# rgcgithub/regenie

Hardware: NVIDIA H100
Metric: step1_level0_snps_per_sec (higher is better)
Workload: dtype int8 Gram + int8 prediction (both exact integer sums) + tf32x3 factorisation + f64 refinement / statistics

## Files before the change

regenie_b200/csrc/chol_mixed.cu:

```cuda
#include <algorithm>

#include "gemm_dmma.cuh"
#include "kernels.cuh"

namespace rg {

namespace {

constexpr int PT = 128;
constexpr int PLD = 132;
constexpr int PB = 32;
constexpr int kMxRowsPerCta = 64;

__device__ __forceinline__ void blk_nt(float (&acc)[PB], const float* __restrict__ Arow, const float* __restrict__ Bt, int plen) {
  for (int p0 = 0; p0 < plen; p0 += 4) {
    const float4 a = *reinterpret_cast<const float4*>(Arow + p0);
#pragma unroll
    for (int n = 0; n < PB; ++n) {
      const float4 b = *reinterpret_cast<const float4*>(Bt + n * PLD + p0);
      acc[n] = fmaf(a.x, b.x, acc[n]);
      acc[n] = fmaf(a.y, b.y, acc[n]);
      acc[n] = fmaf(a.z, b.z, acc[n]);
      acc[n] = fmaf(a.w, b.w, acc[n]);
    }
  }
}

}

__global__ void __launch_bounds__(256)
potrf128_kernel(float* __restrict__ Lplain, float* __restrict__ Mplain, float* __restrict__ MTplain, int n, int k,
                unsigned int* __restrict__ fail_flag) {
  extern __shared__ float pt_sm[];
  float* S = pt_sm;
  float* Wm = pt_sm + PT * PLD;
  float* Wq = pt_sm + 2 * PT * PLD;
  float* dinv = pt_sm + 3 * PT * PLD;
  float* lcol = dinv + PT;
  const int warp = threadIdx.x >> 5, lane = threadIdx.x & 31;
  float* Lkk = Lplain + (int64_t)blockIdx.x * n * n + (int64_t)k * PT * n + (int64_t)k * PT;
#pragma unroll
  for (int it = 0; it < PT * PT / 4 / 256; ++it) {
    const int e = threadIdx.x + 256 * it;
    const int r = e >> 5, c = (e & 31) * 4;
    float4 v = *reinterpret_cast<const float4*>(Lkk + (int64_t)r * n + c);
    if (c + 0 > r) v.x = 0.f;
    if (c + 1 > r) v.y = 0.f;
    if (c + 2 > r) v.z = 0.f;
    if (c + 3 > r) v.w = 0.f;
    *reinterpret_cast<float4*>(S + r * PLD + c) = v;
    *reinterpret_cast<float4*>(Wm + r * PLD + c) = make_float4(0.f, 0.f, 0.f, 0.f);
    *reinterpret_cast<float4*>(Wq + r * PLD + c) = make_float4(0.f, 0.f, 0.f, 0.f);
  }
  __syncthreads();
  bool bad = false;
  for (int jb = 0; jb < PT / PB; ++jb) {
    const int j0 = jb * PB;
    if (warp == 0) {
      float a[PB];
#pragma unroll
      for (int c = 0; c < PB; ++c) a[c] = (c <= lane) ? S[(j0 + lane) * PLD + j0 + c] : 0.f;
      float d = __shfl_sync(0xffffffffu, a[0], 0);
#pragma unroll
      for (int c = 0; c < PB; ++c) {
        if (!(d > 0.f)) bad = true;
        float inv = rsqrtf(d);
        inv = inv * (1.5f - 0.5f * d * inv * inv);
        const float l = a[c] * inv;
        a[c] = l;
        if (lane == c) dinv[j0 + c] = inv;
        if (c + 1 < PB) {
          float* lb = lcol + (c & 1) * PB;
          lb[lane] = l;
          d = __shfl_sync(0xffffffffu, fmaf(-l, l, a[c + 1]), c + 1);
          __syncwarp();
          float lv[PB];
#pragma unroll
          for (int q = (c + 1) / 4; q < PB / 4; ++q) {
            const float4 t4 = *reinterpret_cast<const float4*>(lb + 4 * q);
            lv[4 * q] = t4.x; lv[4 * q + 1] = t4.y; lv[4 * q + 2] = t4.z; lv[4 * q + 3] = t4.w;
          }
#pragma unroll
          for (int cc = c + 1; cc < PB; ++cc) a[cc] = fmaf(-l, lv[cc], a[cc]);
        }
      }
#pragma unroll
      for (int c = 0; c < PB; ++c) S[(j0 + lane) * PLD + j0 + c] = a[c];
    }
    __syncthreads();
    if (warp >= 1 && warp < PT / PB - jb) {
      const int i0 = (jb + warp) * PB;
      float x[PB];
#pragma unroll
      for (int c = 0; c < PB; ++c) x[c] = S[(i0 + lane) * PLD + j0 + c];
#pragma unroll
      for (int c = 0; c < PB; ++c) {
        const float* lrow = S + (j0 + c) * PLD + j0;
        float s = x[c];
#pragma unroll
        for (int p = 0; p < c; ++p) s = fmaf(-x[p], lrow[p], s);
        x[c] = s * dinv[j0 + c];
      }
#pragma unroll
      for (int c = 0; c < PB; ++c) S[(i0 + lane) * PLD + j0 + c] = x[c];
    }
    __syncthreads();
    {
      const int nb = PT / PB - jb - 1;
      int t = 0;
      for (int a1 = 0; a1 < nb; ++a1)
        for (int a2 = 0; a2 <= a1; ++a2, ++t) {
          if ((t & 7) != warp) continue;
          const int ib = jb + 1 + a1, i2 = jb + 1 + a2;
          float acc[PB];
#pragma unroll
          for (int c = 0; c < PB; ++c) acc[c] = 0.f;
          blk_nt(acc, S + (ib * PB + lane) * PLD + j0, S + (i2 * PB) * PLD + j0, PB);
          float* o = S + (ib * PB + lane) * PLD + i2 * PB;
#pragma unroll
          for (int c = 0; c < PB; ++c) o[c] -= acc[c];
        }
    }
    __syncthreads();
  }
  if (bad && lane == 0) atomicOr(fail_flag, 2u);
  if (warp < PT / PB) {
    const int j0 = warp * PB;
    float x[PB];
#pragma unroll
    for (int r = 0; r < PB; ++r) {
      const float* lrow = S + (j0 + r) * PLD + j0;
      float s = (r == lane) ? 1.f : 0.f;
#pragma unroll
      for (int p = 0; p < r; ++p) s = fmaf(-lrow[p], x[p], s);
      x[r] = s * dinv[j0 + r];
    }
#pragma unroll
    for (int r = 0; r < PB; ++r) {
      Wm[(j0 + r) * PLD + j0 + lane] = x[r];
      Wq[(j0 + lane) * PLD + j0 + r] = x[r];
    }
  }
  __syncthreads();
  for (int sb = 1; sb < PT / PB; sb *= 2) {
    const int npair = PT / PB / (2 * sb);
    for (int t = warp; t < npair * sb * sb; t += 8) {
      const int pr = t / (sb * sb), bi = (t / sb) % sb, aj = t % sb;
      const int a0 = pr * 2 * sb, b0 = a0 + sb;
      float acc[PB];
#pragma unroll
      for (int c = 0; c < PB; ++c) acc[c] = 0.f;
      blk_nt(acc, S + ((b0 + bi) * PB + lane) * PLD + (a0 + aj) * PB, Wq + ((a0 + aj) * PB) * PLD + (a0 + aj) * PB, (sb - aj) * PB);
#pragma unroll
      for (int c = 0; c < PB; ++c) S[((a0 + aj) * PB + c) * PLD + (b0 + bi) * PB + lane] = acc[c];
    }
    __syncthreads();
    for (int t = warp; t < npair * sb * sb; t += 8) {
      const int pr = t / (sb * sb), bi = (t / sb) % sb, aj = t % sb;
      const int a0 = pr * 2 * sb, b0 = a0 + sb;
      float acc[PB];
#pragma unroll
      for (int c = 0; c < PB; ++c) acc[c] = 0.f;
      blk_nt(acc, Wm + ((b0 + bi) * PB + lane) * PLD + b0 * PB, S + ((a0 + aj) * PB) * PLD + b0 * PB, (bi + 1) * PB);
#pragma unroll
      for (int c = 0; c < PB; ++c) {
        Wm[((b0 + bi) * PB + lane) * PLD + (a0 + aj) * PB + c] = -acc[c];
        Wq[((a0 + aj) * PB + c) * PLD + (b0 + bi) * PB + lane] = -acc[c];
      }
    }
    __syncthreads();
  }
  float* Mp = Mplain + ((int64_t)blockIdx.x * (n / PT) + k) * PT * PT;
  float* MTp = MTplain + ((int64_t)blockIdx.x * (n / PT) + k) * PT * PT;
#pragma unroll 4
  for (int it = 0; it < PT * PT / 4 / 256; ++it) {
    const int e = threadIdx.x + 256 * it;
    const int r = e >> 5, c = (e & 31) * 4;
    float4 vl = *reinterpret_cast<const float4*>(S + r * PLD + c);
    if (c + 0 > r) vl.x = 0.f;
    if (c + 1 > r) vl.y = 0.f;
    if (c + 2 > r) vl.z = 0.f;
    if (c + 3 > r) vl.w = 0.f;
    *reinterpret_cast<float4*>(Lkk + (int64_t)r * n + c) = vl;
    *reinterpret_cast<float4*>(Mp + r * PT + c) = *reinterpret_cast<const float4*>(Wm + r * PLD + c);
    *reinterpret_cast<float4*>(MTp + r * PT + c) = *reinterpret_cast<const float4*>(Wq + r * PLD + c);
  }
}

constexpr float kMxSafety = 64.f;
__device__ __forceinline__ bool mx_finished(const unsigned int* conv, int nmat, int m, int upto_step, float tol) {
  const bool strict = tol < 0.f;
  const float t = fabsf(tol);
  for (int s = 1; s <= upto_step; ++s) {
    const float dx = __uint_as_float(conv[((int64_t)s * nmat + m) * 2]);
    const float xx = __uint_as_float(conv[((int64_t)s * nmat + m) * 2 + 1]);
    if (dx <= t * xx) return true;
    if (!strict && kMxSafety * dx * dx <= t * xx * xx) return true;
  }
  return false;
}

template <int PMAX>
__global__ void __launch_bounds__(256, 2)
mx_residual_kernel(const double* __restrict__ Af, const double* __restrict__ lambda, int R, const double* __restrict__ bvec,
                   const double* __restrict__ xvec, double* __restrict__ rvec, int n, int P, int Pp, int nmat, int step,
                   const unsigned int* __restrict__ conv, float tol) {
  extern __shared__ double rs_sm[];
  const int m = blockIdx.y;
  if (step > 1 && mx_finished(conv, nmat, m, step - 1, tol)) return;
  const int f = m / R;
  const double lam = lambda[m % R];
  const double* x = xvec + (int64_t)m * Pp * n;
  for (int e = threadIdx.x * 2; e < P * n; e += 512) *reinterpret_cast<double2*>(rs_sm + e) = *reinterpret_cast<const double2*>(x + e);
  __syncthreads();
  const int warp = threadIdx.x >> 5, lane = threadIdx.x & 31;
  for (int rg = 0; rg < kMxRowsPerCta / 32; ++rg) {
  const int i0 = blockIdx.x * kMxRowsPerCta + rg * 32 + warp * 4;
  const double* a0 = Af + ((int64_t)f * n + i0) * n;
  double acc[4][PMAX];
#pragma unroll
  for (int a = 0; a < 4; ++a)
#pragma unroll
    for (int p = 0; p < PMAX; ++p) acc[a][p] = 0.0;
  double2 an2[4];
#pragma unroll
  for (int a = 0; a < 4; ++a) an2[a] = *reinterpret_cast<const double2*>(a0 + (int64_t)a * n + lane * 2);
  for (int j = lane * 2; j < n; j += 64) {
    double2 av[4];
#pragma unroll
    for (int a = 0; a < 4; ++a) av[a] = an2[a];
    if (j + 64 < n) {
#pragma unroll
      for (int a = 0; a < 4; ++a) an2[a] = *reinterpret_cast<const double2*>(a0 + (int64_t)a * n + j + 64);
    }
#pragma unroll
    for (int p = 0; p < PMAX; ++p) {
      if (p < P) {
        const double2 b = *reinterpret_cast<const double2*>(rs_sm + p * n + j);
#pragma unroll
        for (int a = 0; a < 4; ++a) acc[a][p] = fma(av[a].x, b.x, fma(av[a].y, b.y, acc[a][p]));
      }
    }
  }
#pragma unroll
  for (int a = 0; a < 4; ++a)
#pragma unroll
    for (int p = 0; p < PMAX; ++p) {
#pragma unroll
      for (int o = 16; o > 0; o >>= 1) acc[a][p] += __shfl_xor_sync(0xffffffffu, acc[a][p], o);
    }
  if (lane == 0) {
#pragma unroll
    for (int a = 0; a < 4; ++a)
#pragma unroll
      for (int p = 0; p < PMAX; ++p)
        if (p < P)
          rvec[((int64_t)m * Pp + p) * n + i0 + a] = bvec[((int64_t)f * Pp + p) * n + i0 + a] - lam * rs_sm[p * n + i0 + a] - acc[a][p];
  }
  }
}


constexpr int RF_ROWS = 64;
constexpr int RF_NV = 64;

__global__ void __launch_bounds__(256)
mx_residual_fused_kernel(const double* __restrict__ Af, const double* __restrict__ lambda, int R, const double* __restrict__ bvec,
                         const double* __restrict__ xvec, double* __restrict__ rvec, int n, int P, int Pp, int nmat, int step,
                         const unsigned int* __restrict__ conv, float tol) {
  __shared__ double As[64 * DM_LD], Bs[64 * DM_LD];
  const int f = blockIdx.y;
  if (step > 1) {
    bool all_done = true;
    for (int r = 0; r < R; ++r) all_done = all_done && mx_finished(conv, nmat, f * R + r, step - 1, tol);
    if (all_done) return;
  }
  const int NV = R * P;
  const int row0 = blockIdx.x * RF_ROWS;
  const int lrow = threadIdx.x >> 2, lp = (threadIdx.x & 3) * 4;
  const bool vb = lrow < NV;
  const double* ap = Af + ((int64_t)f * n + row0 + lrow) * n + lp;
  const double* bp = xvec + ((int64_t)(f * R + (vb ? lrow / P : 0)) * Pp + (vb ? lrow % P : 0)) * n + lp;
  DmmaAcc acc;
  gemm_tile_nt_dmma_ptr(ap, true, bp, vb, n, acc, As, Bs);
#pragma unroll
  for (int j = 0; j < 4; ++j)
#pragma unroll
    for (int e = 0; e < 2; ++e) {
      const int vec = dm_col(j) + e;
      if (vec < NV) {
        const int r = vec / P, p = vec % P, m = f * R + r;
        const double lam = lambda[r];
#pragma unroll
        for (int i = 0; i < 2; ++i) {
          const int row = row0 + dm_row(i);
          const int64_t o = ((int64_t)m * Pp + p) * n + row;
          rvec[o] = bvec[((int64_t)f * Pp + p) * n + row] - lam * xvec[o] - acc.c[i][j][e];
        }
      }
    }
}

constexpr int TS_STAGES = 6;
constexpr int TS_SUB = 32;
constexpr int TS_STAGE_BYTES = TS_SUB * PT * 4;
constexpr int TS_VP = 12;
constexpr int TS_CW = 16;

__device__ __forceinline__ uint32_t ts_smem_u32(const void* p) { return (uint32_t)__cvta_generic_to_shared(p); }
__device__ __forceinline__ void ts_mbar_wait(uint32_t bar, uint32_t parity) {
  uint32_t done = 0, spins = 0;
  while (true) {
    asm volatile(
        "{\n\t.reg .pred p;\n\t"
        "mbarrier.try_wait.parity.shared::cta.b64 p, [%1], %2;\n\t"
        "selp.u32 %0, 1, 0, p;\n\t}"
        : "=r"(done) : "r"(bar), "r"(parity) : "memory");
    if (done) break;
    if (++spins > (1u << 28)) __trap();
  }
}

template <int PMAX>
__global__ void __launch_bounds__(32 * (TS_CW + 1))
mx_trisolve_kernel(const __grid_constant__ CUtensorMap tmL, const __grid_constant__ CUtensorMap tmM,
                   const __grid_constant__ CUtensorMap tmMT, const double* __restrict__ rvec, int64_t r_mat_stride,
                   int r_mat_div, double* __restrict__ xvec, int n, int P, int Pp, int nmat, int step,
                   unsigned int* __restrict__ conv, float tol) {
  constexpr int TS_PARTS = TS_CW / 4;
  constexpr int TS_CPP = TS_SUB / TS_PARTS;
  constexpr int TS_THREADS = 32 * (TS_CW + 1);
  extern __shared__ uint8_t ts_raw[];
  const int m = blockIdx.x;
  if (step > 1 && mx_finished(conv, nmat, m, step - 1, tol)) return;
  const uint32_t raw = ts_smem_u32(ts_raw);
  const uint32_t base = (raw + 127u) & ~127u;
  uint8_t* gen = ts_raw + (base - raw);
  float* tiles = reinterpret_cast<float*>(gen);
  float* v = reinterpret_cast<float*>(gen + TS_STAGES * TS_STAGE_BYTES);
  float* sbuf = v + (size_t)n * TS_VP;
  float* comb = sbuf + PT * TS_VP;
  uint64_t* bars = reinterpret_cast<uint64_t*>(comb + (TS_PARTS - 1) * PT * TS_VP);
  const uint32_t full_bar = ts_smem_u32(bars), empty_bar = ts_smem_u32(bars + TS_STAGES);
  const int warp = threadIdx.x >> 5, lane = threadIdx.x & 31;
  const int nt = n / PT;
  if (threadIdx.x == 0) {
    for (int s = 0; s < TS_STAGES; ++s) {
      asm volatile("mbarrier.init.shared::cta.b64 [%0], %1;" ::"r"(full_bar + 8 * s), "r"(1) : "memory");
      asm volatile("mbarrier.init.shared::cta.b64 [%0], %1;" ::"r"(empty_bar + 8 * s), "r"(TS_CW) : "memory");
    }
    asm volatile("fence.mbarrier_init.release.cluster;" ::: "memory");
    asm volatile("fence.proxy.async.shared::cta;" ::: "memory");
  }
  const double* r = rvec + (int64_t)(r_mat_div > 0 ? m / r_mat_div : m) * r_mat_stride;
  for (int e = threadIdx.x; e < n * TS_VP; e += TS_THREADS) {
    const int i = e / TS_VP, p = e % TS_VP;
    v[e] = p < P ? (float)r[(int64_t)p * n + i] : 0.f;
  }
  __syncthreads();

  if (warp == TS_CW) {
    if (lane == 0) {
      asm volatile("prefetch.tensormap [%0];" ::"l"(&tmL) : "memory");
      asm volatile("prefetch.tensormap [%0];" ::"l"(&tmM) : "memory");
      asm volatile("prefetch.tensormap [%0];" ::"l"(&tmMT) : "memory");
      int it = 0;
      auto push = [&](const CUtensorMap* tm, int c0, int c1) {
        const int s = it % TS_STAGES;
        const uint32_t ph = (it / TS_STAGES) & 1;
        ts_mbar_wait(empty_bar + 8 * s, ph ^ 1);
        asm volatile("mbarrier.arrive.expect_tx.shared::cta.b64 _, [%0], %1;" ::"r"(full_bar + 8 * s), "r"(TS_STAGE_BYTES) : "memory");
        asm volatile(
            "cp.async.bulk.tensor.2d.shared::cluster.global.mbarrier::complete_tx::bytes [%0], [%1, {%3, %4}], [%2];"
            ::"r"(base + s * TS_STAGE_BYTES), "l"(tm), "r"(full_bar + 8 * s), "r"(c0), "r"(c1) : "memory");
        ++it;
      };
      for (int sweep = 0; sweep < 2; ++sweep)
        for (int kk = 0; kk < nt; ++kk) {
          const int k = sweep == 0 ? kk : nt - 1 - kk;
          const int j0 = sweep == 0 ? 0 : k + 1, j1 = sweep == 0 ? k : nt;
          for (int j = j0; j < j1; ++j)
            for (int sub = 0; sub < PT / TS_SUB; ++sub) push(&tmL, k * PT, m * n + j * PT + sub * TS_SUB);
          for (int sub = 0; sub < PT / TS_SUB; ++sub)
            push(sweep == 0 ? &tmMT : &tmM, 0, (m * nt + k) * PT + sub * TS_SUB);
        }
    }
    return;
  }

  const int half = warp >> 2;
  const int row = (warp & 3) * 32 + lane;
  int it = 0;
  float acc[PMAX];
  auto consume = [&](const float* vec ) {
    const int s = it % TS_STAGES;
    const uint32_t ph = (it / TS_STAGES) & 1;
    ts_mbar_wait(full_bar + 8 * s, ph);
    const float* t = tiles + (size_t)s * (TS_STAGE_BYTES / 4) + (size_t)(half * TS_CPP) * PT + row;
    const float* y = vec + (size_t)(half * TS_CPP) * TS_VP;
#pragma unroll
    for (int c = 0; c < TS_CPP; ++c) {
      const float tv = t[(size_t)c * PT];
      const float4 y0 = *reinterpret_cast<const float4*>(y + c * TS_VP);
      const float4 y1 = *reinterpret_cast<const float4*>(y + c * TS_VP + 4);
      const float4 y2 = *reinterpret_cast<const float4*>(y + c * TS_VP + 8);
      const float yy[12] = {y0.x, y0.y, y0.z, y0.w, y1.x, y1.y, y1.z, y1.w, y2.x, y2.y, y2.z, y2.w};
#pragma unroll
      for (int p = 0; p < PMAX; ++p) acc[p] = fmaf(tv, yy[p], acc[p]);
    }
    __syncwarp();
    if (lane == 0) asm volatile("mbarrier.arrive.shared::cta.b64 _, [%0];" ::"r"(empty_bar + 8 * s) : "memory");
    ++it;
  };
  auto consumer_sync = [&]() { asm volatile("bar.sync 1, %0;" ::"n"(32 * TS_CW) : "memory"); };

  for (int sweep = 0; sweep < 2; ++sweep)
    for (int kk = 0; kk < nt; ++kk) {
      const int k = sweep == 0 ? kk : nt - 1 - kk;
      const int j0 = sweep == 0 ? 0 : k + 1, j1 = sweep == 0 ? k : nt;
#pragma unroll
      for (int p = 0; p < PMAX; ++p) acc[p] = 0.f;
      for (int j = j0; j < j1; ++j)
        for (int sub = 0; sub < PT / TS_SUB; ++sub) consume(v + (size_t)(j * PT + sub * TS_SUB) * TS_VP);
      if (half > 0) {
#pragma unroll
        for (int p = 0; p < PMAX; ++p) comb[((half - 1) * PT + row) * TS_VP + p] = acc[p];
      }
      consumer_sync();
      if (half == 0) {
#pragma unroll
        for (int p = 0; p < PMAX; ++p) {
          float sum = acc[p];
#pragma unroll
          for (int h = 0; h < TS_PARTS - 1; ++h) sum += comb[(h * PT + row) * TS_VP + p];
          sbuf[row * TS_VP + p] = v[(size_t)(k * PT + row) * TS_VP + p] - sum;
        }
      }
      consumer_sync();
#pragma unroll
      for (int p = 0; p < PMAX; ++p) acc[p] = 0.f;
      for (int sub = 0; sub < PT / TS_SUB; ++sub) consume(sbuf + (size_t)(sub * TS_SUB) * TS_VP);
      if (half > 0) {
#pragma unroll
        for (int p = 0; p < PMAX; ++p) comb[((half - 1) * PT + row) * TS_VP + p] = acc[p];
      }
      consumer_sync();
      if (half == 0) {
#pragma unroll
        for (int p = 0; p < PMAX; ++p) {
          float sum = acc[p];
#pragma unroll
          for (int h = 0; h < TS_PARTS - 1; ++h) sum += comb[(h * PT + row) * TS_VP + p];
          v[(size_t)(k * PT + row) * TS_VP + p] = sum;
        }
      }
      consumer_sync();
    }

  float dmax = 0.f, xmax = 0.f;
  for (int e = threadIdx.x; e < P * n; e += 32 * TS_CW) {
    const int p = e / n, i = e % n;
    double* xp = xvec + ((int64_t)m * Pp + p) * n + i;
    const float dx = v[(size_t)i * TS_VP + p];
    const double xn = (step == 0 ? 0.0 : *xp) + (double)dx;
    *xp = xn;
    dmax = (fabsf(dx) <= 3.0e38f) ? fmaxf(dmax, fabsf(dx)) : __int_as_float(0x7f800000);
    xmax = fmaxf(xmax, fabsf((float)xn));
  }
  if (step > 0) {
#pragma unroll
    for (int o = 16; o > 0; o >>= 1) {
      dmax = fmaxf(dmax, __shfl_xor_sync(0xffffffffu, dmax, o));
      xmax = fmaxf(xmax, __shfl_xor_sync(0xffffffffu, xmax, o));
    }
    if (lane == 0) {
      atomicMax(conv + ((int64_t)step * nmat + m) * 2, __float_as_uint(dmax));
      atomicMax(conv + ((int64_t)step * nmat + m) * 2 + 1, __float_as_uint(xmax));
    }
  }
}

__global__ void mx_final_check_kernel(const unsigned int* __restrict__ conv, int nmat, int steps, float tol,
                                      unsigned int* __restrict__ fail_flag) {
  const int m = blockIdx.x * blockDim.x + threadIdx.x;
  if (m >= nmat) return;
  bool ok = mx_finished(conv, nmat, m, steps, tol);
  for (int s = 1; s <= steps; ++s) {
    const float dx = __uint_as_float(conv[((int64_t)s * nmat + m) * 2]);
    if (!(dx == dx) || !(fabsf(dx) <= 3.0e38f)) ok = false;
  }
  if (!ok) atomicOr(fail_flag, 1u);
}

struct MxPlan {
  int n = 0, nt = 0;
  DevBuf<int4> tiles;
  std::vector<int2> upd, trsm;
};

static void build_plan(MxPlan& pl, int n) {
  pl.n = n;
  const int nt = n / PT;
  pl.nt = nt;
  std::vector<int4> all;
  pl.upd.clear(); pl.trsm.clear();
  for (int k = 0; k < nt; ++k) {
    int2 u{(int)all.size(), 0};
    for (int i = k; i < nt; ++i) all.push_back(make_int4(i, k, 0, 4 * k));
    u.y = (int)all.size() - u.x;
    pl.upd.push_back(u);
    int2 t{(int)all.size(), 0};
    for (int i = k + 1; i < nt; ++i) all.push_back(make_int4(i, k, 4 * k, 4));
    t.y = (int)all.size() - t.x;
    pl.trsm.push_back(t);
  }
  pl.tiles.alloc(all.size());
  RG_CUDA(cudaMemcpy(pl.tiles.p, all.data(), all.size() * sizeof(int4), cudaMemcpyHostToDevice));
}

struct MixedSolver::Impl {
  int n = 0, nmat = 0, K = 0, R = 0, Pp = 0;
  DevBuf<float> Lplain, Mplain, MTplain, Ap;
  DevBuf<unsigned int> conv;
  CUtensorMap tmL, tmM, tmAp;
  CUtensorMap tmLpl, tmMpl, tmMTpl;
  MxPlan plan;
};

MixedSolver::MixedSolver() : impl(new Impl()) {}
MixedSolver::~MixedSolver() { delete impl; }

int MixedSolver::dim_for(int bs) {
  int n = PT;
  while (n < bs) n *= 2;
  return n <= 2048 ? n : 0;
}

void MixedSolver::prepare(int n, int K, int R, int Pp) {
  Impl& d = *impl;
  const int nmat = K * R;
  if (d.n == n && d.nmat == nmat && d.Pp == Pp) return;
  RG_CHECK(n % PT == 0 && n >= PT && ((n / PT) & (n / PT - 1)) == 0 && n <= 2048,
           "mixed solver: dimension must be 128 * 2^k <= 2048");
  d.n = n; d.nmat = nmat; d.K = K; d.R = R; d.Pp = Pp;
  d.Lplain.alloc((size_t)nmat * n * n);
  d.Mplain.alloc((size_t)nmat * n * PT);
  d.MTplain.alloc((size_t)nmat * n * PT);
  make_f32_rows_tensor_map(&d.tmLpl, d.Lplain.p, n, (int64_t)nmat * n, PT, TS_SUB);
  make_f32_rows_tensor_map(&d.tmMpl, d.Mplain.p, PT, (int64_t)nmat * n, PT, TS_SUB);
  make_f32_rows_tensor_map(&d.tmMTpl, d.MTplain.p, PT, (int64_t)nmat * n, PT, TS_SUB);
  RG_CUDA(cudaMemset(d.Lplain.p, 0, (size_t)nmat * n * n * 4));
  d.conv.alloc((size_t)(kMxMaxSteps + 1) * nmat * 2);
  make_tf32_operand_tensor_map(&d.tmL, d.Lplain.p, n, n, nmat);
  make_tf32_operand_tensor_map(&d.tmM, d.Mplain.p, PT, n, nmat);
  d.Ap.alloc((size_t)K * n * n);
  RG_CUDA(cudaMemset(d.Ap.p, 0, (size_t)K * n * n * 4));
  make_tf32_operand_tensor_map(&d.tmAp, d.Ap.p, n, n, K);
  build_plan(d.plan, n);
}

static int rhs_chunk(int n) { return std::max(1, std::min(12, (int)(98304 / (8 * (size_t)n)))); }

int MixedSolver::launches_per_solve(int n, int steps, int P) {
  const int nt = n / PT;
  const int nch = (P + rhs_chunk(n) - 1) / rhs_chunk(n);
  return 3 * nt - 1 + nch * (1 + 2 * steps) + 1;
}

void MixedSolver::solve(const double* Af, const double* lambda, const double* bvec, double* xvec, double* rvec, int P,
                        int steps, float tol, unsigned int* fail_flag, cudaStream_t s, bool first_col_ready) {
  Impl& d = *impl;
  const int n = d.n, nmat = d.nmat, nt = d.plan.nt;
  RG_CHECK(n > 0, "mixed solver: prepare() first");
  RG_CHECK(P <= d.Pp, "mixed solver: more right-hand sides than the row pitch");
  RG_CHECK(steps >= 1 && steps <= kMxMaxSteps, "mixed solver: bad step count");
  const size_t potrf_smem = ((size_t)3 * PT * PLD + PT + 2 * PB) * sizeof(float);
  ensure_dyn_smem(reinterpret_cast<const void*>(potrf128_kernel), potrf_smem);
  ensure_dyn_smem(reinterpret_cast<const void*>(mx_residual_kernel<12>), 98304);
  ensure_dyn_smem(reinterpret_cast<const void*>(mx_residual_kernel<10>), 98304);
  RG_CHECK(n <= 2048, "mixed solver: n <= 2048");
  const size_t sm_t = (size_t)TS_STAGES * TS_STAGE_BYTES + ((size_t)n + (1 + TS_CW / 4) * PT) * TS_VP * sizeof(float) + 2 * TS_STAGES * 8 + 256;
  ensure_dyn_smem(reinterpret_cast<const void*>(mx_trisolve_kernel<12>), sm_t);
  ensure_dyn_smem(reinterpret_cast<const void*>(mx_trisolve_kernel<10>), sm_t);
  RG_CUDA(cudaMemsetAsync(d.conv.p, 0, d.conv.n * sizeof(unsigned int), s));
  const int4* tl = d.plan.tiles.p;
  Tf32GemmEpilogue e0{};
  e0.n = n; e0.out_mat_stride = (int64_t)n * n; e0.out = d.Lplain.p;
  for (int k = 0; k < nt; ++k) {
    Tf32GemmEpilogue e = e0;
    e.c_chunks = 4; e.c_mat_div = d.R;
    e.diag_add = lambda; e.diag_mod = d.R;
    if (!(k == 0 && first_col_ready)) launch_tf32x3_gemm(d.tmL, d.tmL, tl + d.plan.upd[k].x, d.plan.upd[k].y, nmat, e, s, &d.tmAp);
    potrf128_kernel<<<nmat, 256, potrf_smem, s>>>(d.Lplain.p, d.Mplain.p, d.MTplain.p, n, k, fail_flag);
    if (d.plan.trsm[k].y > 0) {
      Tf32GemmEpilogue t = e0;
      t.mirror = 1;
      t.b_cols_local = 1;
      launch_tf32x3_gemm(d.tmL, d.tmM, tl + d.plan.trsm[k].x, d.plan.trsm[k].y, nmat, t, s);
    }
  }
  dim3 grid(n / kMxRowsPerCta, nmat);
  const int pc = rhs_chunk(n);
  for (int st = 0; st <= steps; ++st)
    for (int p0 = 0; p0 < P; p0 += pc) {
      const int np = std::min(pc, P - p0);
      const size_t sm_r = (size_t)np * n * sizeof(double);
      const int64_t o = (int64_t)p0 * n;
      auto tri = [&](const double* rv, int64_t rs, int rdiv, int step) {
#define RG_TRI(PM) mx_trisolve_kernel<PM><<<nmat, 32 * (TS_CW + 1), sm_t, s>>>(d.tmLpl, d.tmMpl, d.tmMTpl, rv, rs, rdiv, xvec + o, n, np, d.Pp, nmat, step, d.conv.p, tol)
        if (np <= 10) RG_TRI(10);
        else RG_TRI(12);
#undef RG_TRI
      };
      if (st == 0) {
        tri(bvec + o, (int64_t)d.Pp * n, d.R, 0);
      } else {
        if (d.R * np <= RF_NV && n % RF_ROWS == 0)
          mx_residual_fused_kernel<<<dim3(n / RF_ROWS, d.K), 256, 0, s>>>(Af, lambda, d.R, bvec + o, xvec + o, rvec + o, n, np, d.Pp, nmat, st, d.conv.p, tol);
        else if (np <= 10) mx_residual_kernel<10><<<grid, 256, sm_r, s>>>(Af, lambda, d.R, bvec + o, xvec + o, rvec + o, n, np, d.Pp, nmat, st, d.conv.p, tol);
        else mx_residual_kernel<12><<<grid, 256, sm_r, s>>>(Af, lambda, d.R, bvec + o, xvec + o, rvec + o, n, np, d.Pp, nmat, st, d.conv.p, tol);
        tri(rvec + o, (int64_t)d.Pp * n, 0, st);
      }
    }
  mx_final_check_kernel<<<(nmat + 63) / 64, 64, 0, s>>>(d.conv.p, nmat, steps, tol, fail_flag);
}

float* MixedSolver::a_planes() { return impl->Ap.p; }
float* MixedSolver::l_planes() { return impl->Lplain.p; }

const float* MixedSolver::debug_planes(int which) const {
  switch (which) {
    case 2: return impl->Lplain.p;
    case 3: return impl->Mplain.p;
    default: return nullptr;
  }
}

}
```

Baseline: 999,700.

## Restructure triangular solve kernel: fewer warps, 4-row register tiles, two CTAs per SM

The TMA-fed triangular solve now uses 4 consumer warps instead of 16. Each thread accumulates 4 rows times PMAX right-hand sides using float4 tile loads, and a shared reduction buffer combines the per-warp partial sums. Stage count is chosen at runtime so that two CTAs fit per SM, which comes with launch_bounds min-blocks=2, and the vector pitch shrinks from 12 to PMAX. Load/store loops now use shift/mask indexing, which assumes n is a power of two. In exchange, each thread uses more registers, and the smaller pipeline depth could expose latency.

```diff
diff --git a/regenie_b200/csrc/chol_mixed.cu b/regenie_b200/csrc/chol_mixed.cu
--- a/regenie_b200/csrc/chol_mixed.cu
+++ b/regenie_b200/csrc/chol_mixed.cu
@@ -301,11 +301,12 @@
     }
 }
 
-constexpr int TS_STAGES = 6;
+constexpr int TS_MAX_STAGES = 6;
 constexpr int TS_SUB = 32;
 constexpr int TS_STAGE_BYTES = TS_SUB * PT * 4;
-constexpr int TS_VP = 12;
-constexpr int TS_CW = 16;
+constexpr int TS_CW = 4;
+constexpr int TS_CPP = TS_SUB / TS_CW;
+constexpr int TS_THREADS = 32 * (TS_CW + 1);
 
 __device__ __forceinline__ uint32_t ts_smem_u32(const void* p) { return (uint32_t)__cvta_generic_to_shared(p); }
 __device__ __forceinline__ void ts_mbar_wait(uint32_t bar, uint32_t parity) {
@@ -322,14 +323,14 @@
 }
 
 template <int PMAX>
-__global__ void __launch_bounds__(32 * (TS_CW + 1))
+__global__ void __launch_bounds__(TS_THREADS, 2)
 mx_trisolve_kernel(const __grid_constant__ CUtensorMap tmL, const __grid_constant__ CUtensorMap tmM,
                    const __grid_constant__ CUtensorMap tmMT, const double* __restrict__ rvec, int64_t r_mat_stride,
                    int r_mat_div, double* __restrict__ xvec, int n, int P, int Pp, int nmat, int step,
-                   unsigned int* __restrict__ conv, float tol) {
-  constexpr int TS_PARTS = TS_CW / 4;
-  constexpr int TS_CPP = TS_SUB / TS_PARTS;
-  constexpr int TS_THREADS = 32 * (TS_CW + 1);
+                   unsigned int* __restrict__ conv, float tol, int stages) {
+  constexpr int VP = PMAX;
+  constexpr int CG = VP % 4 == 0 ? 1 : 2;
+  static_assert((CG * VP) % 4 == 0 && TS_CPP % CG == 0 && (TS_CPP * VP) % 4 == 0, "16-byte aligned vector row groups");
   extern __shared__ uint8_t ts_raw[];
   const int m = blockIdx.x;
   if (step > 1 && mx_finished(conv, nmat, m, step - 1, tol)) return;
@@ -337,15 +338,15 @@
   const uint32_t base = (raw + 127u) & ~127u;
   uint8_t* gen = ts_raw + (base - raw);
   float* tiles = reinterpret_cast<float*>(gen);
-  float* v = reinterpret_cast<float*>(gen + TS_STAGES * TS_STAGE_BYTES);
-  float* sbuf = v + (size_t)n * TS_VP;
-  float* comb = sbuf + PT * TS_VP;
-  uint64_t* bars = reinterpret_cast<uint64_t*>(comb + (TS_PARTS - 1) * PT * TS_VP);
-  const uint32_t full_bar = ts_smem_u32(bars), empty_bar = ts_smem_u32(bars + TS_STAGES);
+  float* v = reinterpret_cast<float*>(gen + (size_t)stages * TS_STAGE_BYTES);
+  float* part = v + (size_t)n * VP;
+  uint64_t* bars = reinterpret_cast<uint64_t*>(part + TS_CW * PT * VP);
+  const uint32_t full_bar = ts_smem_u32(bars), empty_bar = ts_smem_u32(bars + stages);
   const int warp = threadIdx.x >> 5, lane = threadIdx.x & 31;
   const int nt = n / PT;
+  const int lg_n = __ffs(n) - 1;
   if (threadIdx.x == 0) {
-    for (int s = 0; s < TS_STAGES; ++s) {
+    for (int s = 0; s < stages; ++s) {
       asm volatile("mbarrier.init.shared::cta.b64 [%0], %1;" ::"r"(full_bar + 8 * s), "r"(1) : "memory");
       asm volatile("mbarrier.init.shared::cta.b64 [%0], %1;" ::"r"(empty_bar + 8 * s), "r"(TS_CW) : "memory");
     }
@@ -353,10 +354,9 @@
     asm volatile("fence.proxy.async.shared::cta;" ::: "memory");
   }
   const double* r = rvec + (int64_t)(r_mat_div > 0 ? m / r_mat_div : m) * r_mat_stride;
-  for (int e = threadIdx.x; e < n * TS_VP; e += TS_THREADS) {
-    const int i = e / TS_VP, p = e % TS_VP;
-    v[e] = p < P ? (float)r[(int64_t)p * n + i] : 0.f;
-  }
+#pragma unroll 4
+  for (int e = threadIdx.x; e < P * n; e += TS_THREADS) v[(e & (n - 1)) * VP + (e >> lg_n)] = (float)r[e];
+  for (int e = threadIdx.x; e < (VP - P) * n; e += TS_THREADS) v[(e & (n - 1)) * VP + P + (e >> lg_n)] = 0.f;
   __syncthreads();
 
   if (warp == TS_CW) {
@@ -364,16 +364,15 @@
       asm volatile("prefetch.tensormap [%0];" ::"l"(&tmL) : "memory");
       asm volatile("prefetch.tensormap [%0];" ::"l"(&tmM) : "memory");
       asm volatile("prefetch.tensormap [%0];" ::"l"(&tmMT) : "memory");
-      int it = 0;
+      int s = 0;
+      uint32_t ph = 0;
       auto push = [&](const CUtensorMap* tm, int c0, int c1) {
-        const int s = it % TS_STAGES;
-        const uint32_t ph = (it / TS_STAGES) & 1;
         ts_mbar_wait(empty_bar + 8 * s, ph ^ 1);
         asm volatile("mbarrier.arrive.expect_tx.shared::cta.b64 _, [%0], %1;" ::"r"(full_bar + 8 * s), "r"(TS_STAGE_BYTES) : "memory");
         asm volatile(
             "cp.async.bulk.tensor.2d.shared::cluster.global.mbarrier::complete_tx::bytes [%0], [%1, {%3, %4}], [%2];"
             ::"r"(base + s * TS_STAGE_BYTES), "l"(tm), "r"(full_bar + 8 * s), "r"(c0), "r"(c1) : "memory");
-        ++it;
+        if (++s == stages) { s = 0; ph ^= 1; }
       };
       for (int sweep = 0; sweep < 2; ++sweep)
         for (int kk = 0; kk < nt; ++kk) {
@@ -388,84 +387,109 @@
     return;
   }
 
-  const int half = warp >> 2;
-  const int row = (warp & 3) * 32 + lane;
-  int it = 0;
-  float acc[PMAX];
+  int s = 0;
+  uint32_t ph = 0;
+  float acc[4][PMAX];
   auto consume = [&](const float* vec ) {
-    const int s = it % TS_STAGES;
-    const uint32_t ph = (it / TS_STAGES) & 1;
     ts_mbar_wait(full_bar + 8 * s, ph);
-    const float* t = tiles + (size_t)s * (TS_STAGE_BYTES / 4) + (size_t)(half * TS_CPP) * PT + row;
-    const float* y = vec + (size_t)(half * TS_CPP) * TS_VP;
-#pragma unroll
-    for (int c = 0; c < TS_CPP; ++c) {
-      const float tv = t[(size_t)c * PT];
-      const float4 y0 = *reinterpret_cast<const float4*>(y + c * TS_VP);
-      const float4 y1 = *reinterpret_cast<const float4*>(y + c * TS_VP + 4);
-      const float4 y2 = *reinterpret_cast<const float4*>(y + c * TS_VP + 8);
-      const float yy[12] = {y0.x, y0.y, y0.z, y0.w, y1.x, y1.y, y1.z, y1.w, y2.x, y2.y, y2.z, y2.w};
-#pragma unroll
-      for (int p = 0; p < PMAX; ++p) acc[p] = fmaf(tv, yy[p], acc[p]);
+    const float4* t = reinterpret_cast<const float4*>(tiles + (size_t)s * (TS_STAGE_BYTES / 4) + (size_t)(warp * TS_CPP) * PT) + lane;
+    const float4* y = reinterpret_cast<const float4*>(vec + (size_t)(warp * TS_CPP) * VP);
+#pragma unroll
+    for (int c = 0; c < TS_CPP; c += CG) {
+      float yy[CG * VP];
+#pragma unroll
+      for (int q = 0; q < CG * VP / 4; ++q) {
+        const float4 y4 = y[c * VP / 4 + q];
+        yy[4 * q] = y4.x; yy[4 * q + 1] = y4.y; yy[4 * q + 2] = y4.z; yy[4 * q + 3] = y4.w;
+      }
+#pragma unroll
+      for (int h = 0; h < CG; ++h) {
+        const float4 t4 = t[(c + h) * (PT / 4)];
+        const float tv[4] = {t4.x, t4.y, t4.z, t4.w};
+#pragma unroll
+        for (int a = 0; a < 4; ++a)
+#pragma unroll
+          for (int p = 0; p < PMAX; ++p) acc[a][p] = fmaf(tv[a], yy[h * VP + p], acc[a][p]);
+      }
     }
     __syncwarp();
     if (lane == 0) asm volatile("mbarrier.arrive.shared::cta.b64 _, [%0];" ::"r"(empty_bar + 8 * s) : "memory");
-    ++it;
+    if (++s == stages) { s = 0; ph ^= 1; }
   };
   auto consumer_sync = [&]() { asm volatile("bar.sync 1, %0;" ::"n"(32 * TS_CW) : "memory"); };
+  auto zero = [&]() {
+#pragma unroll
+    for (int a = 0; a < 4; ++a)
+#pragma unroll
+      for (int p = 0; p < PMAX; ++p) acc[a][p] = 0.f;
+  };
+  auto reduce_into = [&](float* blk, bool subtract) {
+    float4* pw = reinterpret_cast<float4*>(part + (size_t)(warp * PT + 4 * lane) * VP);
+#pragma unroll
+    for (int q = 0; q < VP; ++q) {
+      const int f = 4 * q;
+      float w[4];
+#pragma unroll
+      for (int u = 0; u < 4; ++u) w[u] = acc[(f + u) / VP][(f + u) % VP];
+      pw[q] = make_float4(w[0], w[1], w[2], w[3]);
+    }
+    consumer_sync();
+    for (int e = threadIdx.x; e < PT * VP / 4; e += 32 * TS_CW) {
+      const float4* pr = reinterpret_cast<const float4*>(part) + e;
+      float4 sum = pr[0];
+#pragma unroll
+      for (int h = 1; h < TS_CW; ++h) {
+        const float4 o = pr[h * (PT * VP / 4)];
+        sum.x += o.x; sum.y += o.y; sum.z += o.z; sum.w += o.w;
+      }
+      float4* d = reinterpret_cast<float4*>(blk) + e;
+      if (subtract) {
+        const float4 b = *d;
+        sum = make_float4(b.x - sum.x, b.y - sum.y, b.z - sum.z, b.w - sum.w);
+      }
+      *d = sum;
+    }
+    consumer_sync();
+  };
 
   for (int sweep = 0; sweep < 2; ++sweep)
     for (int kk = 0; kk < nt; ++kk) {
       const int k = sweep == 0 ? kk : nt - 1 - kk;
       const int j0 = sweep == 0 ? 0 : k + 1, j1 = sweep == 0 ? k : nt;
-#pragma unroll
-      for (int p = 0; p < PMAX; ++p) acc[p] = 0.f;
-      for (int j = j0; j < j1; ++j)
-        for (int sub = 0; sub < PT / TS_SUB; ++sub) consume(v + (size_t)(j * PT + sub * TS_SUB) * TS_VP);
-      if (half > 0) {
-#pragma unroll
-        for (int p = 0; p < PMAX; ++p) comb[((half - 1) * PT + row) * TS_VP + p] = acc[p];
-      }
-      consumer_sync();
-      if (half == 0) {
-#pragma unroll
-        for (int p = 0; p < PMAX; ++p) {
-          float sum = acc[p];
-#pragma unroll
-          for (int h = 0; h < TS_PARTS - 1; ++h) sum += comb[(h * PT + row) * TS_VP + p];
-          sbuf[row * TS_VP + p] = v[(size_t)(k * PT + row) * TS_VP + p] - sum;
-        }
-      }
-      consumer_sync();
-#pragma unroll
-      for (int p = 0; p < PMAX; ++p) acc[p] = 0.f;
-      for (int sub = 0; sub < PT / TS_SUB; ++sub) consume(sbuf + (size_t)(sub * TS_SUB) * TS_VP);
-      if (half > 0) {
-#pragma unroll
-        for (int p = 0; p < PMAX; ++p) comb[((half - 1) * PT + row) * TS_VP + p] = acc[p];
-      }
-      consumer_sync();
-      if (half == 0) {
-#pragma unroll
-        for (int p = 0; p < PMAX; ++p) {
-          float sum = acc[p];
-#pragma unroll
-          for (int h = 0; h < TS_PARTS - 1; ++h) sum += comb[(h * PT + row) * TS_VP + p];
-          v[(size_t)(k * PT + row) * TS_VP + p] = sum;
-        }
-      }
-      consumer_sync();
+      float* vk = v + (size_t)k * PT * VP;
+      if (j1 > j0) {
+        zero();
+        for (int j = j0; j < j1; ++j)
+          for (int sub = 0; sub < PT / TS_SUB; ++sub) consume(v + (size_t)(j * PT + sub * TS_SUB) * VP);
+        reduce_into(vk, true);
+      }
+      zero();
+      for (int sub = 0; sub < PT / TS_SUB; ++sub) consume(vk + (size_t)(sub * TS_SUB) * VP);
+      reduce_into(vk, false);
     }
 
   float dmax = 0.f, xmax = 0.f;
-  for (int e = threadIdx.x; e < P * n; e += 32 * TS_CW) {
-    const int p = e / n, i = e % n;
-    double* xp = xvec + ((int64_t)m * Pp + p) * n + i;
-    const float dx = v[(size_t)i * TS_VP + p];
-    const double xn = (step == 0 ? 0.0 : *xp) + (double)dx;
-    *xp = xn;
-    dmax = (fabsf(dx) <= 3.0e38f) ? fmaxf(dmax, fabsf(dx)) : __int_as_float(0x7f800000);
-    xmax = fmaxf(xmax, fabsf((float)xn));
+  double* x = xvec + (int64_t)m * Pp * n;
+  constexpr int XB = 4;
+  for (int e0 = threadIdx.x; e0 < P * n; e0 += XB * 32 * TS_CW) {
+    double xo[XB];
+#pragma unroll
+    for (int u = 0; u < XB; ++u) {
+      const int e = e0 + u * 32 * TS_CW;
+      xo[u] = (step == 0 || e >= P * n) ? 0.0 : x[(int64_t)(e >> lg_n) * n + (e & (n - 1))];
+    }
+#pragma unroll
+    for (int u = 0; u < XB; ++u) {
+      const int e = e0 + u * 32 * TS_CW;
+      if (e < P * n) {
+        const int p = e >> lg_n, i = e & (n - 1);
+        const float dx = v[(size_t)i * VP + p];
+        const double xn = xo[u] + (double)dx;
+        x[(int64_t)p * n + i] = xn;
+        dmax = (fabsf(dx) <= 3.0e38f) ? fmaxf(dmax, fabsf(dx)) : __int_as_float(0x7f800000);
+        xmax = fmaxf(xmax, fabsf((float)xn));
+      }
+    }
   }
   if (step > 0) {
 #pragma unroll
@@ -559,6 +583,17 @@
   build_plan(d.plan, n);
 }
 
+static size_t trisolve_smem(int n, int pmax, int stages) {
+  return (size_t)stages * TS_STAGE_BYTES + ((size_t)n + TS_CW * PT) * pmax * sizeof(float) + 2 * (size_t)stages * 8 + 128;
+}
+
+static int trisolve_stages(int n, int pmax) {
+  constexpr size_t kTwoPerSm = 228 * 1024 / 2 - 1024;
+  for (int st = TS_MAX_STAGES; st >= 3; --st)
+    if (trisolve_smem(n, pmax, st) <= kTwoPerSm) return st;
+  return TS_MAX_STAGES;
+}
+
 static int rhs_chunk(int n) { return std::max(1, std::min(12, (int)(98304 / (8 * (size_t)n)))); }
 
 int MixedSolver::launches_per_solve(int n, int steps, int P) {
@@ -579,9 +614,6 @@
   ensure_dyn_smem(reinterpret_cast<const void*>(mx_residual_kernel<12>), 98304);
   ensure_dyn_smem(reinterpret_cast<const void*>(mx_residual_kernel<10>), 98304);
   RG_CHECK(n <= 2048, "mixed solver: n <= 2048");
-  const size_t sm_t = (size_t)TS_STAGES * TS_STAGE_BYTES + ((size_t)n + (1 + TS_CW / 4) * PT) * TS_VP * sizeof(float) + 2 * TS_STAGES * 8 + 256;
-  ensure_dyn_smem(reinterpret_cast<const void*>(mx_trisolve_kernel<12>), sm_t);
-  ensure_dyn_smem(reinterpret_cast<const void*>(mx_trisolve_kernel<10>), sm_t);
   RG_CUDA(cudaMemsetAsync(d.conv.p, 0, d.conv.n * sizeof(unsigned int), s));
   const int4* tl = d.plan.tiles.p;
   Tf32GemmEpilogue e0{};
@@ -607,7 +639,14 @@
       const size_t sm_r = (size_t)np * n * sizeof(double);
       const int64_t o = (int64_t)p0 * n;
       auto tri = [&](const double* rv, int64_t rs, int rdiv, int step) {
-#define RG_TRI(PM) mx_trisolve_kernel<PM><<<nmat, 32 * (TS_CW + 1), sm_t, s>>>(d.tmLpl, d.tmMpl, d.tmMTpl, rv, rs, rdiv, xvec + o, n, np, d.Pp, nmat, step, d.conv.p, tol)
+#define RG_TRI(PM)                                                                                                       \
+  do {                                                                                                                   \
+    const int stages = trisolve_stages(n, PM);                                                                           \
+    const size_t sm_t = trisolve_smem(n, PM, stages);                                                                    \
+    ensure_dyn_smem(reinterpret_cast<const void*>(mx_trisolve_kernel<PM>), sm_t);                                        \
+    mx_trisolve_kernel<PM><<<nmat, TS_THREADS, sm_t, s>>>(d.tmLpl, d.tmMpl, d.tmMTpl, rv, rs, rdiv, xvec + o, n, np,     \
+                                                        d.Pp, nmat, step, d.conv.p, tol, stages);                      \
+  } while (0)
         if (np <= 10) RG_TRI(10);
         else RG_TRI(12);
 #undef RG_TRI
```

Result: faster. 1.017 million (median of 6 runs) (+1.7%).
